# pengsongyou/openscene

Hardware: AMD Instinct MI355X
Metric: active voxels/sec MinkUNet18A fwd+bwd @2cm ScanNet; per-point query ms (higher is better)
Workload: dtype f32 (bf16x6 split-precision MFMA, fp32 accumulate); 1 GPU; ScanNet distillation step (configs[2]): MinkUNet18A, 768-d head, 1 synthetic S100k scene/GPU (100999 voxels on rank 0, 2 cm), training-mode BN; timed = coordinate+kernel maps, forward, cosine loss, backward, gradient all-reduce, Adam step; arch=MinkUNet18A, feature_dim=768, voxels_rank0=100999, parallelism=dp1

## Files before the change

### openscene_amd/csrc/bn.hip

```cpp
#include "common.h"
#include "epilogue.h"

namespace osn {

constexpr int CR_COLS = 64;
constexpr int CR_RL = 16;
constexpr int CR_MAX_BLOCKS = 512;

constexpr int BN_MAX_SRC = 3;
struct GySrc {
    const float* p[BN_MAX_SRC];
    int64_t ld[BN_MAX_SRC];
    int n;
};

__device__ inline float4 gy_load(const GySrc& s, int64_t r, int col) {
    float4 g = *reinterpret_cast<const float4*>(s.p[0] + r * s.ld[0] + col);
#pragma unroll
    for (int i = 1; i < BN_MAX_SRC; ++i)
        if (i < s.n) {
            const float4 v = *reinterpret_cast<const float4*>(s.p[i] + r * s.ld[i] + col);
            g.x += v.x; g.y += v.y; g.z += v.z; g.w += v.w;
        }
    return g;
}


struct ColReducePlan {
    int n_rb;
    int n_cg;
    int rows_per_block;
};

static ColReducePlan plan_colreduce(int64_t n, int c) {
    ColReducePlan p;
    p.n_cg = int(cdiv(c, CR_COLS));
    int64_t rb = cdiv(n, 4 * CR_RL);
    if (rb > CR_MAX_BLOCKS) rb = CR_MAX_BLOCKS;
    if (rb < 1) rb = 1;
    p.rows_per_block = int(cdiv(cdiv(n, rb), CR_RL) * CR_RL);
    p.n_rb = int(cdiv(n, p.rows_per_block));
    if (p.n_rb < 1) p.n_rb = 1;
    return p;
}

template <int MODE>
__global__ __launch_bounds__(256) void col_reduce_kernel(const float* __restrict__ x, const float* __restrict__ y,
                                                         const GySrc gy, const float* __restrict__ mean,
                                                         const float* __restrict__ var, float eps, int relu, int64_t n,
                                                         int c, int rows_per_block, double* __restrict__ partial,
                                                         const float* __restrict__ gamma, const float* __restrict__ beta) {
    __shared__ double red[2][CR_RL][CR_COLS];
    const int tid = threadIdx.x;
    const int cl = tid & 15, rl = tid >> 4;
    const int col = blockIdx.y * CR_COLS + cl * 4;
    const bool on = col < c;
    const int64_t r0 = int64_t(blockIdx.x) * rows_per_block;
    const int64_t r1 = min(n, r0 + rows_per_block);
    double s1[4] = {0, 0, 0, 0}, s2[4] = {0, 0, 0, 0};
    float4 mu = make_float4(0, 0, 0, 0), is = make_float4(0, 0, 0, 0);
    float4 ga = make_float4(0, 0, 0, 0), be = make_float4(0, 0, 0, 0);
    const bool from_x = MODE == 1 && relu && !y;
    if (MODE == 1 && on) {
        mu = *reinterpret_cast<const float4*>(mean + col);
        const float4 v = *reinterpret_cast<const float4*>(var + col);
        is = make_float4(bn_is(v.x, eps), bn_is(v.y, eps), bn_is(v.z, eps), bn_is(v.w, eps));
        if (from_x) {
            ga = *reinterpret_cast<const float4*>(gamma + col);
            be = *reinterpret_cast<const float4*>(beta + col);
        }
    }
    if (on) {
        for (int64_t r = r0 + rl; r < r1; r += CR_RL) {
            const float4 xv = *reinterpret_cast<const float4*>(x + r * c + col);
            if (MODE == 0) {
                s1[0] += xv.x; s1[1] += xv.y; s1[2] += xv.z; s1[3] += xv.w;
                s2[0] += double(xv.x) * xv.x; s2[1] += double(xv.y) * xv.y;
                s2[2] += double(xv.z) * xv.z; s2[3] += double(xv.w) * xv.w;
            } else {
                float4 g = gy_load(gy, r, col);
                if (from_x) {
                    g.x = bn_val(xv.x, mu.x, is.x, ga.x, be.x) > 0.f ? g.x : 0.f;
                    g.y = bn_val(xv.y, mu.y, is.y, ga.y, be.y) > 0.f ? g.y : 0.f;
                    g.z = bn_val(xv.z, mu.z, is.z, ga.z, be.z) > 0.f ? g.z : 0.f;
                    g.w = bn_val(xv.w, mu.w, is.w, ga.w, be.w) > 0.f ? g.w : 0.f;
                } else if (relu) {
                    const float4 yv = *reinterpret_cast<const float4*>(y + r * c + col);
                    g.x = yv.x > 0.f ? g.x : 0.f; g.y = yv.y > 0.f ? g.y : 0.f;
                    g.z = yv.z > 0.f ? g.z : 0.f; g.w = yv.w > 0.f ? g.w : 0.f;
                }
                s1[0] += g.x; s1[1] += g.y; s1[2] += g.z; s1[3] += g.w;
                s2[0] += double(g.x) * ((xv.x - mu.x) * is.x); s2[1] += double(g.y) * ((xv.y - mu.y) * is.y);
                s2[2] += double(g.z) * ((xv.z - mu.z) * is.z); s2[3] += double(g.w) * ((xv.w - mu.w) * is.w);
            }
        }
    }
#pragma unroll
    for (int j = 0; j < 4; ++j) {
        red[0][rl][cl * 4 + j] = s1[j];
        red[1][rl][cl * 4 + j] = s2[j];
    }
    __syncthreads();
    if (tid < 2 * CR_COLS) {
        const int which = tid / CR_COLS, cc = tid % CR_COLS;
        double s = 0;
#pragma unroll
        for (int r = 0; r < CR_RL; ++r) s += red[which][r][cc];
        const int gc = blockIdx.y * CR_COLS + cc;
        if (gc < c) partial[(int64_t(blockIdx.x) * 2 + which) * c + gc] = s;
    }
}

constexpr int FIN_COLS = 16, FIN_PARTS = 64;

constexpr int FIN_ITERS = CR_MAX_BLOCKS / FIN_PARTS;

__device__ inline void finalize_sums(const double* __restrict__ partial, int n_rb, int c, double& s1, double& s2,
                                     int& col) {
    __shared__ double red[2][FIN_PARTS][FIN_COLS];
    const int cl = threadIdx.x & (FIN_COLS - 1), part = threadIdx.x / FIN_COLS;
    col = blockIdx.x * FIN_COLS + cl;
    double va[FIN_ITERS], vb[FIN_ITERS];
    const int cc = col < c ? col : 0;
#pragma unroll
    for (int i = 0; i < FIN_ITERS; ++i) {
        const int blk = part + FIN_PARTS * i;
        const int bc = blk < n_rb ? blk : 0;
        va[i] = partial[(int64_t(bc) * 2 + 0) * c + cc];
        vb[i] = partial[(int64_t(bc) * 2 + 1) * c + cc];
    }
    double a = 0, b = 0;
#pragma unroll
    for (int i = 0; i < FIN_ITERS; ++i) {
        const bool on = col < c && part + FIN_PARTS * i < n_rb;
        a += on ? va[i] : 0.0;
        b += on ? vb[i] : 0.0;
    }
    red[0][part][cl] = a;
    red[1][part][cl] = b;
    __syncthreads();
    double t1 = 0, t2 = 0;
    if (part < 8) {
#pragma unroll
        for (int q = 0; q < 8; ++q) { t1 += red[0][part * 8 + q][cl]; t2 += red[1][part * 8 + q][cl]; }
    }
    __syncthreads();
    if (part < 8) {
        red[0][part][cl] = t1;
        red[1][part][cl] = t2;
    }
    __syncthreads();
    s1 = 0; s2 = 0;
    if (part == 0) {
#pragma unroll
        for (int q = 0; q < 8; ++q) { s1 += red[0][q][cl]; s2 += red[1][q][cl]; }
    }
}

__global__ __launch_bounds__(FIN_COLS * FIN_PARTS) void bn_stats_finalize_kernel(
    const double* __restrict__ partial, int n_rb, int64_t n, int c, float* __restrict__ mean, float* __restrict__ var,
    float* __restrict__ running_mean, float* __restrict__ running_var, float momentum) {
    double s1, s2;
    int j;
    finalize_sums(partial, n_rb, c, s1, s2, j);
    if (threadIdx.x >= FIN_COLS || j >= c) return;
    const double m = s1 / double(n);
    double v = s2 / double(n) - m * m;
    if (v < 0) v = 0;
    mean[j] = float(m);
    var[j] = float(v);
    if (running_mean) running_mean[j] = (1.f - momentum) * running_mean[j] + momentum * float(m);
    if (running_var) {
        const double unb = n > 1 ? v * double(n) / double(n - 1) : v;
        running_var[j] = (1.f - momentum) * running_var[j] + momentum * float(unb);
    }
}

__global__ __launch_bounds__(FIN_COLS * FIN_PARTS) void bn_bwd_finalize_kernel(const double* __restrict__ partial,
                                                                              int n_rb, int c,
                                                                              float* __restrict__ sum_g,
                                                                              float* __restrict__ sum_gx) {
    double s1, s2;
    int j;
    finalize_sums(partial, n_rb, c, s1, s2, j);
    if (threadIdx.x >= FIN_COLS || j >= c) return;
    sum_g[j] = float(s1);
    sum_gx[j] = float(s2);
}

__device__ inline float4 ld4(const float* p) { return *reinterpret_cast<const float4*>(p); }


__global__ __launch_bounds__(256) void bn_apply_kernel(const float* __restrict__ x, const float* __restrict__ mean,
                                                       const float* __restrict__ var, const float* __restrict__ gamma,
                                                       const float* __restrict__ beta, float eps,
                                                       const float* __restrict__ residual, int relu,
                                                       float* __restrict__ y, float* __restrict__ y2, int64_t ld2,
                                                       int64_t total4, int c4) {
    for (int64_t e = int64_t(blockIdx.x) * blockDim.x + threadIdx.x; e < total4; e += int64_t(gridDim.x) * blockDim.x) {
        const int col = int(e % c4) * 4;
        const float4 xv = ld4(x + e * 4), mu = ld4(mean + col), vv = ld4(var + col), ga = ld4(gamma + col),
                     be = ld4(beta + col);
        float4 o;
        o.x = bn_val(xv.x, mu.x, bn_is(vv.x, eps), ga.x, be.x);
        o.y = bn_val(xv.y, mu.y, bn_is(vv.y, eps), ga.y, be.y);
        o.z = bn_val(xv.z, mu.z, bn_is(vv.z, eps), ga.z, be.z);
        o.w = bn_val(xv.w, mu.w, bn_is(vv.w, eps), ga.w, be.w);
        if (residual) {
            const float4 rv = ld4(residual + e * 4);
            o.x += rv.x; o.y += rv.y; o.z += rv.z; o.w += rv.w;
        }
        if (relu) {
            o.x = bn_relu(o.x); o.y = bn_relu(o.y); o.z = bn_relu(o.z); o.w = bn_relu(o.w);
        }
        *reinterpret_cast<float4*>(y + e * 4) = o;
        if (y2) *reinterpret_cast<float4*>(y2 + (e / c4) * ld2 + col) = o;
    }
}

__global__ __launch_bounds__(256) void bn_bwd_apply_kernel(const float* __restrict__ x, const float* __restrict__ y,
                                                           const GySrc gy, const float* __restrict__ mean,
                                                           const float* __restrict__ var, const float* __restrict__ gamma,
                                                           float eps, int relu, int training,
                                                           const float* __restrict__ sum_g,
                                                           const float* __restrict__ sum_gx, float inv_n,
                                                           float* __restrict__ gx, float* __restrict__ gres,
                                                           int64_t total4, int c4, const float* __restrict__ beta) {
    const bool from_x = relu && !y;
    for (int64_t e = int64_t(blockIdx.x) * blockDim.x + threadIdx.x; e < total4; e += int64_t(gridDim.x) * blockDim.x) {
        const int col = int(e % c4) * 4;
        float4 g = gy_load(gy, e / c4, col);
        const float4 vv = ld4(var + col), ga = ld4(gamma + col);
        const float4 is = make_float4(bn_is(vv.x, eps), bn_is(vv.y, eps), bn_is(vv.z, eps), bn_is(vv.w, eps));
        float4 xv = make_float4(0, 0, 0, 0), mu = make_float4(0, 0, 0, 0);
        if (training || from_x) { xv = ld4(x + e * 4); mu = ld4(mean + col); }
        if (from_x) {
            const float4 be = ld4(beta + col);
            g.x = bn_val(xv.x, mu.x, is.x, ga.x, be.x) > 0.f ? g.x : 0.f;
            g.y = bn_val(xv.y, mu.y, is.y, ga.y, be.y) > 0.f ? g.y : 0.f;
            g.z = bn_val(xv.z, mu.z, is.z, ga.z, be.z) > 0.f ? g.z : 0.f;
            g.w = bn_val(xv.w, mu.w, is.w, ga.w, be.w) > 0.f ? g.w : 0.f;
        } else if (relu) {
            const float4 yv = ld4(y + e * 4);
            g.x = yv.x > 0.f ? g.x : 0.f; g.y = yv.y > 0.f ? g.y : 0.f;
            g.z = yv.z > 0.f ? g.z : 0.f; g.w = yv.w > 0.f ? g.w : 0.f;
        }
        if (gres) *reinterpret_cast<float4*>(gres + e * 4) = g;
        float4 o;
        if (training) {
            const float4 sg = ld4(sum_g + col), sx = ld4(sum_gx + col);
            o.x = ga.x * is.x * (g.x - sg.x * inv_n - (xv.x - mu.x) * is.x * sx.x * inv_n);
            o.y = ga.y * is.y * (g.y - sg.y * inv_n - (xv.y - mu.y) * is.y * sx.y * inv_n);
            o.z = ga.z * is.z * (g.z - sg.z * inv_n - (xv.z - mu.z) * is.z * sx.z * inv_n);
            o.w = ga.w * is.w * (g.w - sg.w * inv_n - (xv.w - mu.w) * is.w * sx.w * inv_n);
        } else {
            o.x = ga.x * is.x * g.x; o.y = ga.y * is.y * g.y; o.z = ga.z * is.z * g.z; o.w = ga.w * is.w * g.w;
        }
        *reinterpret_cast<float4*>(gx + e * 4) = o;
    }
}

constexpr int SB_THREADS = 1024, SB_RL = 512, SB_PER = 8, SB_COLS = 8;
constexpr int SB_MAX_ROWS = SB_RL * SB_PER;

__device__ inline double sb_wave_sum(double v) {
#pragma unroll
    for (int off = 2; off < 64; off <<= 1) v += __shfl_xor(v, off, 64);
    return v;
}

__device__ inline void sb_block_sums(double (&s)[8], int tid, int cl) {
    __shared__ double red[SB_THREADS / 64][2][8];
    __shared__ double tot[2][8];
#pragma unroll
    for (int q = 0; q < 8; ++q) s[q] = sb_wave_sum(s[q]);
    const int lane = tid & 63, wave = tid >> 6;
    if ((lane >> 1) == 0) {
#pragma unroll
        for (int q = 0; q < 8; ++q) red[wave][cl][q] = s[q];
    }
    __syncthreads();
    if (tid < 16) {
        const int c2 = tid >> 3, q = tid & 7;
        double t = 0;
#pragma unroll
        for (int w = 0; w < SB_THREADS / 64; ++w) t += red[w][c2][q];
        tot[c2][q] = t;
    }
    __syncthreads();
#pragma unroll
    for (int q = 0; q < 8; ++q) s[q] = tot[cl][q];
}

__global__ __launch_bounds__(SB_THREADS) void bn_small_fwd_kernel(const float* __restrict__ x, int n, int c,
                                                                  const float* __restrict__ gamma, const float* __restrict__ beta,
                                                                  float eps, const float* __restrict__ residual, int relu,
                                                                  float momentum, float* __restrict__ mean_out,
                                                                  float* __restrict__ var_out, float* __restrict__ running_mean,
                                                                  float* __restrict__ running_var, float* __restrict__ y,
                                                                  float* __restrict__ y2, int64_t ld2) {
    const int tid = threadIdx.x, cl = tid & 1, rl = tid >> 1;
    const int col = blockIdx.x * SB_COLS + cl * 4;
    const bool con = col < c;
    const int cc = con ? col : 0;
    float4 v[SB_PER];
    double s[8] = {0, 0, 0, 0, 0, 0, 0, 0};
#pragma unroll
    for (int j = 0; j < SB_PER; ++j) {
        const int r = rl + SB_RL * j;
        const bool ok = con && r < n;
        v[j] = ld4(x + int64_t(ok ? r : 0) * c + cc);
        if (ok) {
            s[0] += v[j].x; s[1] += v[j].y; s[2] += v[j].z; s[3] += v[j].w;
            s[4] += double(v[j].x) * v[j].x; s[5] += double(v[j].y) * v[j].y;
            s[6] += double(v[j].z) * v[j].z; s[7] += double(v[j].w) * v[j].w;
        }
    }
    sb_block_sums(s, tid, cl);
    float mu[4], vr[4];
#pragma unroll
    for (int q = 0; q < 4; ++q) {
        const double m = s[q] / double(n);
        double var = s[4 + q] / double(n) - m * m;
        if (var < 0) var = 0;
        mu[q] = float(m);
        vr[q] = float(var);
        if (rl == 0 && con) {
            mean_out[col + q] = mu[q];
            var_out[col + q] = vr[q];
            if (running_mean) running_mean[col + q] = (1.f - momentum) * running_mean[col + q] + momentum * mu[q];
            if (running_var) {
                const double unb = n > 1 ? var * double(n) / double(n - 1) : var;
                running_var[col + q] = (1.f - momentum) * running_var[col + q] + momentum * float(unb);
            }
        }
    }
    if (!con) return;
    const float4 ga = ld4(gamma + col), be = ld4(beta + col);
    const float is0 = bn_is(vr[0], eps), is1 = bn_is(vr[1], eps), is2 = bn_is(vr[2], eps), is3 = bn_is(vr[3], eps);
#pragma unroll
    for (int j = 0; j < SB_PER; ++j) {
        const int r = rl + SB_RL * j;
        if (r >= n) continue;
        float4 o;
        o.x = bn_val(v[j].x, mu[0], is0, ga.x, be.x);
        o.y = bn_val(v[j].y, mu[1], is1, ga.y, be.y);
        o.z = bn_val(v[j].z, mu[2], is2, ga.z, be.z);
        o.w = bn_val(v[j].w, mu[3], is3, ga.w, be.w);
        if (residual) {
            const float4 rv = ld4(residual + int64_t(r) * c + col);
            o.x += rv.x; o.y += rv.y; o.z += rv.z; o.w += rv.w;
        }
        if (relu) {
            o.x = bn_relu(o.x); o.y = bn_relu(o.y); o.z = bn_relu(o.z); o.w = bn_relu(o.w);
        }
        *reinterpret_cast<float4*>(y + int64_t(r) * c + col) = o;
        if (y2) *reinterpret_cast<float4*>(y2 + int64_t(r) * ld2 + col) = o;
    }
}

static int ew_grid(int64_t total4) {
    int64_t g = cdiv(total4, 256);
    if (g > 2048) g = 2048;
    if (g < 1) g = 1;
    return int(g);
}

}

using namespace osn;

extern "C" size_t osn_bn_ws_bytes(int64_t n, int c) {
    (void)n;
    return size_t(CR_MAX_BLOCKS) * 2 * size_t(c) * 8 + 256;
}

extern "C" int osn_bn_stats(const float* x, int64_t n, int c, float* mean, float* var, float* running_mean,
                            float* running_var, float momentum, void* ws, size_t ws_bytes, osn_stream_t stream) {
    hipStream_t st = static_cast<hipStream_t>(stream);
    OSN_REQUIRE(n >= 1 && c >= 4 && (c & 3) == 0, OSN_E_ARG, "osn_bn_stats: need n >= 1 and c %% 4 == 0 (n=%lld c=%d)", (long long)n, c);
    OSN_REQUIRE(x && mean && var && aligned16(x), OSN_E_ARG, "osn_bn_stats: null or unaligned pointer");
    ColReducePlan p = plan_colreduce(n, c);
    const size_t need = size_t(p.n_rb) * 2 * size_t(c) * 8;
    OSN_REQUIRE(ws && ws_bytes >= need, OSN_E_WS, "osn_bn_stats: workspace %zu < %zu", ws_bytes, need);
    double* partial = static_cast<double*>(ws);
    hipLaunchKernelGGL((col_reduce_kernel<0>), dim3(p.n_rb, p.n_cg), dim3(256), 0, st, x, (const float*)nullptr,
                       GySrc{}, (const float*)nullptr, (const float*)nullptr, 0.f, 0, n, c,
                       p.rows_per_block, partial, (const float*)nullptr, (const float*)nullptr);
    hipLaunchKernelGGL(bn_stats_finalize_kernel, dim3(cdiv(c, FIN_COLS)), dim3(FIN_COLS * FIN_PARTS), 0, st, partial, p.n_rb, n, c, mean, var,
                       running_mean, running_var, momentum);
    OSN_LAUNCH_CHECK();
    return OSN_OK;
}

extern "C" int osn_bn_apply2(const float* x, const float* mean, const float* var, const float* gamma, const float* beta,
                             float eps, const float* residual, int relu, float* y, float* y2, int64_t ld2, int64_t n, int c,
                             osn_stream_t stream) {
    hipStream_t st = static_cast<hipStream_t>(stream);
    OSN_REQUIRE(n >= 0 && c >= 4 && (c & 3) == 0, OSN_E_ARG, "osn_bn_apply: need c %% 4 == 0 (c=%d)", c);
    if (n == 0) return OSN_OK;
    OSN_REQUIRE(x && mean && var && gamma && beta && y, OSN_E_ARG, "osn_bn_apply: null pointer");
    OSN_REQUIRE(aligned16(x) && aligned16(y) && aligned16(mean) && aligned16(var) && aligned16(gamma) && aligned16(beta) &&
                    (!residual || aligned16(residual)),
                OSN_E_ARG, "osn_bn_apply: pointers must be 16-byte aligned");
    OSN_REQUIRE(!y2 || (aligned16(y2) && ld2 >= c && (ld2 & 3) == 0), OSN_E_ARG,
                "osn_bn_apply2: the second destination needs a 16-byte aligned pointer and a row stride >= c, %% 4 == 0");
    const int64_t total4 = n * (c / 4);
    hipLaunchKernelGGL(bn_apply_kernel, dim3(ew_grid(total4)), dim3(256), 0, st, x, mean, var, gamma, beta, eps,
                       residual, relu, y, y2, ld2, total4, c / 4);
    OSN_LAUNCH_CHECK();
    return OSN_OK;
}

extern "C" int osn_bn_apply(const float* x, const float* mean, const float* var, const float* gamma, const float* beta,
                            float eps, const float* residual, int relu, float* y, int64_t n, int c,
                            osn_stream_t stream) {
    return osn_bn_apply2(x, mean, var, gamma, beta, eps, residual, relu, y, nullptr, 0, n, c, stream);
}

extern "C" int osn_bn_forward_train2(const float* x, int64_t n, int c, const float* gamma, const float* beta, float eps,
                                     const float* residual, int relu, float momentum, float* mean, float* var,
                                     float* running_mean, float* running_var, float* y, float* y2, int64_t ld2, void* ws,
                                     size_t ws_bytes, osn_stream_t stream) {
    if (n >= 1 && n <= SB_MAX_ROWS && c >= 4 && (c & 3) == 0) {
        hipStream_t st = static_cast<hipStream_t>(stream);
        OSN_REQUIRE(x && mean && var && gamma && beta && y, OSN_E_ARG, "osn_bn_forward_train: null pointer");
        OSN_REQUIRE(aligned16(x) && aligned16(y) && aligned16(gamma) && aligned16(beta) && (!residual || aligned16(residual)),
                    OSN_E_ARG, "osn_bn_forward_train: pointers must be 16-byte aligned");
        OSN_REQUIRE(!y2 || (aligned16(y2) && ld2 >= c && (ld2 & 3) == 0), OSN_E_ARG,
                    "osn_bn_forward_train2: the second destination needs a 16-byte aligned pointer and a row stride >= c, %% 4 == 0");
        hipLaunchKernelGGL(bn_small_fwd_kernel, dim3(unsigned(cdiv(c, SB_COLS))), dim3(SB_THREADS), 0, st, x, int(n), c, gamma,
                           beta, eps, residual, relu, momentum, mean, var, running_mean, running_var, y, y2, ld2);
        OSN_LAUNCH_CHECK();
        return OSN_OK;
    }
    int rc = osn_bn_stats(x, n, c, mean, var, running_mean, running_var, momentum, ws, ws_bytes, stream);
    if (rc) return rc;
    return osn_bn_apply2(x, mean, var, gamma, beta, eps, residual, relu, y, y2, ld2, n, c, stream);
}

extern "C" int osn_bn_forward_train(const float* x, int64_t n, int c, const float* gamma, const float* beta, float eps,
                                    const float* residual, int relu, float momentum, float* mean, float* var,
                                    float* running_mean, float* running_var, float* y, void* ws, size_t ws_bytes,
                                    osn_stream_t stream) {
    return osn_bn_forward_train2(x, n, c, gamma, beta, eps, residual, relu, momentum, mean, var, running_mean, running_var, y,
                                 nullptr, 0, ws, ws_bytes, stream);
}

extern "C" int osn_bn_backward_multi2(const float* x, const float* y, const float* const* gy, const int64_t* gy_ld, int n_gy,
                                      const float* mean, const float* var, const float* gamma, const float* beta, float eps, int relu,
                                     int training, float* gx, float* gres, float* ggamma, float* gbeta, int64_t n, int c,
                                     void* ws, size_t ws_bytes, osn_stream_t stream) {
    hipStream_t st = static_cast<hipStream_t>(stream);
    OSN_REQUIRE(n >= 1 && c >= 4 && (c & 3) == 0, OSN_E_ARG, "osn_bn_backward: need n >= 1 and c %% 4 == 0");
    OSN_REQUIRE(gy && gy_ld && n_gy >= 1 && n_gy <= BN_MAX_SRC, OSN_E_ARG,
                "osn_bn_backward: %d gradient sources (1 .. %d are supported)", n_gy, BN_MAX_SRC);
    OSN_REQUIRE(x && mean && var && gamma && gx && ggamma && gbeta && (!relu || y || beta), OSN_E_ARG,
                "osn_bn_backward: null pointer");
    OSN_REQUIRE(!(relu && !y) || !gres, OSN_E_ARG, "osn_bn_backward: the ReLU mask can be recomputed from x only without a residual");
    OSN_REQUIRE(!beta || aligned16(beta), OSN_E_ARG, "osn_bn_backward: beta must be 16-byte aligned");
    OSN_REQUIRE(aligned16(x) && aligned16(gx) && aligned16(mean) && aligned16(var) && aligned16(gamma) &&
                    aligned16(ggamma) && aligned16(gbeta) && (!y || aligned16(y)) && (!gres || aligned16(gres)),
                OSN_E_ARG, "osn_bn_backward: pointers must be 16-byte aligned");
    GySrc src{};
    src.n = n_gy;
    for (int i = 0; i < BN_MAX_SRC; ++i) {
        const int j = i < n_gy ? i : 0;
        OSN_REQUIRE(gy[j] && aligned16(gy[j]) && gy_ld[j] >= c && (gy_ld[j] & 3) == 0, OSN_E_ARG,
                    "osn_bn_backward: gradient source %d needs a 16-byte aligned pointer and a row stride >= c, %% 4 == 0", j);
        src.p[i] = gy[j];
        src.ld[i] = gy_ld[j];
    }
    ColReducePlan p = plan_colreduce(n, c);
    const size_t need = size_t(p.n_rb) * 2 * size_t(c) * 8;
    OSN_REQUIRE(ws && ws_bytes >= need, OSN_E_WS, "osn_bn_backward: workspace %zu < %zu", ws_bytes, need);
    double* partial = static_cast<double*>(ws);
    hipLaunchKernelGGL((col_reduce_kernel<1>), dim3(p.n_rb, p.n_cg), dim3(256), 0, st, x, y, src, mean, var, eps, relu, n,
                       c, p.rows_per_block, partial, gamma, beta);
    hipLaunchKernelGGL(bn_bwd_finalize_kernel, dim3(cdiv(c, FIN_COLS)), dim3(FIN_COLS * FIN_PARTS), 0, st, partial, p.n_rb, c, gbeta, ggamma);
    const int64_t total4 = n * (c / 4);
    hipLaunchKernelGGL(bn_bwd_apply_kernel, dim3(ew_grid(total4)), dim3(256), 0, st, x, y, src, mean, var, gamma, eps,
                       relu, training, gbeta, ggamma, 1.f / float(n), gx, gres, total4, c / 4, beta);
    OSN_LAUNCH_CHECK();
    return OSN_OK;
}

extern "C" int osn_bn_backward_multi(const float* x, const float* y, const float* const* gy, const int64_t* gy_ld, int n_gy,
                                     const float* mean, const float* var, const float* gamma, float eps, int relu,
                                     int training, float* gx, float* gres, float* ggamma, float* gbeta, int64_t n, int c,
                                     void* ws, size_t ws_bytes, osn_stream_t stream) {
    OSN_REQUIRE(!relu || y, OSN_E_ARG, "osn_bn_backward_multi: relu needs y (or osn_bn_backward_multi2 with beta)");
    return osn_bn_backward_multi2(x, y, gy, gy_ld, n_gy, mean, var, gamma, nullptr, eps, relu, training, gx, gres, ggamma, gbeta, n, c,
                                  ws, ws_bytes, stream);
}

extern "C" int osn_bn_backward(const float* x, const float* y, const float* gy, const float* mean, const float* var,
                               const float* gamma, float eps, int relu, int training, float* gx, float* gres,
                               float* ggamma, float* gbeta, int64_t n, int c, void* ws, size_t ws_bytes,
                               osn_stream_t stream) {
    const int64_t ld = c;
    return osn_bn_backward_multi(x, y, &gy, &ld, 1, mean, var, gamma, eps, relu, training, gx, gres, ggamma, gbeta, n, c, ws,
                                 ws_bytes, stream);
}
```

### openscene_amd/csrc/net.hip

```cpp
#include "common.h"
#include <stdlib.h>
#include "events.h"
#include "epilogue.h"
#include <vector>

namespace osn {

constexpr uint64_t NO_OFF = ~uint64_t(0);

struct Events {
    std::vector<hipEvent_t> ev;
};

int events_count(const osn_events_t* e) { return e ? int(reinterpret_cast<const Events*>(e)->ev.size()) : 0; }
hipEvent_t events_get(const osn_events_t* e, int i) { return reinterpret_cast<const Events*>(e)->ev[size_t(i)]; }

struct Prof {
    std::vector<hipEvent_t> ev;
    std::vector<int32_t> tag;
    std::vector<int32_t> only;
    int cap = 0, n = 0;
};

static inline uint64_t up256(uint64_t x) { return (x + 255) & ~uint64_t(255); }
// ... 390 lines not shown
            OSN_HIP(hipEventRecord(evs->ev[net->n_ops + 1 + i], side));
            pending[i] = 1;
        }
    }
    for (int i = run->first_op; i < run->end_op; ++i)
        if (pending[i]) OSN_HIP(hipStreamWaitEvent(st, evs->ev[net->n_ops + 1 + i], 0));
    return OSN_OK;
}

extern "C" int osn_net_backward(const osn_net_desc* net, const osn_net_run* run, osn_stream_t stream) {
    OSN_REQUIRE(net && run, OSN_E_ARG, "osn_net_backward: null argument");
    Layout L;
    int rc = make_layout(net, run->level_rows, 1, L);
    if (rc) return rc;
    rc = check_run(net, run, L, true);
    if (rc) return rc;
    hipStream_t st = static_cast<hipStream_t>(stream);
    char* A = static_cast<char*>(run->fwd_arena);
    char* B = static_cast<char*>(run->bwd_arena);
    const int64_t* rows = run->level_rows;
    std::vector<osn_wgrad_job> jobs;
    jobs.reserve(size_t(net->n_ops));
    Events* evs = reinterpret_cast<Events*>(run->events);
    hipStream_t side = static_cast<hipStream_t>(run->side_stream);
    const bool forked = side && side != st && evs && int(evs->ev.size()) >= 2 * net->n_ops + 2 && run->ws_side &&
                        run->ws_side_bytes >= L.ws_bytes;
    osn_stream_t wstream = forked ? run->side_stream : stream;
    void* wws = forked ? run->ws_side : run->ws;
    const size_t wws_bytes = size_t(forked ? run->ws_side_bytes : run->ws_bytes);
    for (int i = run->end_op - 1; i >= run->first_op; --i) {
        const osn_net_op& o = net->ops[i];
        const int64_t n_in = rows[o.lvl_in], n_out = rows[o.lvl_out];
        const osn_net_weight& w = run->weights[o.weight];
        const float* gsrc[4];
        int64_t gld[4];
        int ng = 0;
        if (o.dst < 0) {
            OSN_REQUIRE(run->goutput || (run->goutput_rows && run->grows_pos && run->grows_idx && run->n_grows > 0), OSN_E_ARG,
                        "osn_net_backward: null output gradient");
            gsrc[ng] = run->goutput; gld[ng] = o.cout; ++ng;
        } else {
            for (int j = i + 1; j < net->n_ops && ng < 4; ++j) {
                const osn_net_op& c = net->ops[j];
                if (c.src == o.dst && c.need_dgrad) { gsrc[ng] = reinterpret_cast<const float*>(B + L.gin_off[j]); gld[ng] = c.cin; ++ng; }
                if (ng < 4 && c.res == o.dst) { gsrc[ng] = reinterpret_cast<const float*>(B + L.gres_off[j]); gld[ng] = c.cout; ++ng; }
                if (ng < 4 && o.copy_buf >= 0 && c.src == o.copy_buf && c.need_dgrad) {
                    gsrc[ng] = reinterpret_cast<const float*>(B + L.gin_off[j]) + o.copy_col; gld[ng] = c.cin; ++ng;
                }
            }
            OSN_REQUIRE(ng >= 1 && ng <= 3, OSN_E_ARG, "osn_net_backward: the output of op %d has %s consumers inside the executed range (1 .. 3 supported)",
                        i, ng == 0 ? "no" : "more than three");
        }
        const osn_net_run* r = run;
        const osn_stream_t sstream = stream;
        const float* gx;
        if (o.bn >= 0) {
            const osn_net_bn& bn = run->bns[o.bn];
            const float* x = reinterpret_cast<const float*>(A + L.x_off[i]);
            const float* y = reinterpret_cast<const float*>(A + L.y_off[o.dst]);
            const float *mean = bn.running_mean, *var = bn.running_var;
            if (run->training) {
                const float* mv = reinterpret_cast<const float*>(A + L.stat_off[i]);
                mean = mv; var = mv + o.cout;
            }
            float* gxw = reinterpret_cast<float*>(B + L.gx_off[i]);
            float* gres = o.res >= 0 ? reinterpret_cast<float*>(B + L.gres_off[i]) : nullptr;
            OSN_REQUIRE(bn.ggamma && bn.gbeta, OSN_E_ARG, "osn_net_backward: op %d: null batch-norm gradient pointers", i);
            const bool from_x = o.relu && o.res < 0 && bn.beta;
            rc = osn_bn_backward_multi2(x, from_x ? nullptr : y, gsrc, gld, ng, mean, var, bn.gamma, from_x ? bn.beta : nullptr, bn.eps,
                                        o.relu, run->training, gxw, gres, bn.ggamma, bn.gbeta, n_out, o.cout, r->ws, size_t(r->ws_bytes),
                                        sstream);
            if (rc) return rc;
            gx = gxw;
        } else {
            OSN_REQUIRE(ng == 1 && gld[0] == o.cout, OSN_E_ARG, "osn_net_backward: op %d without a batch norm needs one contiguous gradient", i);
            gx = gsrc[0];
        }
        const float* in = o.src < 0 ? run->input : reinterpret_cast<const float*>(A + L.y_off[o.src]);
        MapView v{};
        const osn_net_map* m = o.map >= 0 ? &run->maps[o.map] : nullptr;
        if (m) v = view_of(*m, o.transposed != 0);
        const bool sparse_rows = o.dst < 0 && o.K == 1 && o.bn < 0 && run->goutput_rows && run->grows_pos && run->grows_idx &&
                                 run->n_grows > 0 && run->n_grows < n_out && L.rows_in_off != NO_OFF &&
                                 (L.wgrad_k[i] == OSN_NET_K_WGRAD || L.wgrad_k[i] == OSN_NET_K_WGRAD_TL) &&
                                 (!o.need_dgrad || L.dgrad_k[i] == OSN_NET_K_DENSE);
        OSN_REQUIRE(o.dst >= 0 || sparse_rows || run->goutput, OSN_E_ARG,
                    "osn_net_backward: op %d: only the supervised rows of the output gradient were given, but the row-compacted head "
                    "backward does not apply to this configuration", i);
        OSN_REQUIRE(w.gW, OSN_E_ARG, "osn_net_backward: op %d: null weight-gradient pointer", i);
        if (forked && L.wgrad_k[i] == OSN_NET_K_WGRAD_STEM && !jobs.empty()) {
            rc = osn_wgrad_tl_reduce_batch(jobs.data(), int(jobs.size()), wstream);
            jobs.clear();
            if (rc) return rc;
        }
        const bool wg_main = forked && L.wgrad_k[i] == OSN_NET_K_WGRAD_STEM;
        if (forked && !wg_main) {
            OSN_HIP(hipEventRecord(evs->ev[i], st));
            OSN_HIP(hipStreamWaitEvent(side, evs->ev[i], 0));
        }
        {
            Bracket br(run->prof, i, 2, (forked && !wg_main) ? side : st);
            if (sparse_rows) {
                float* in_rows = reinterpret_cast<float*>(B + L.rows_in_off);
                rc = osn_rows_gather(in, run->grows_idx, run->n_grows, o.cin, in_rows, wstream);
                if (!rc)
                    rc = osn_spconv_wgrad(in_rows, run->goutput_rows, nullptr, nullptr, nullptr, w.gW, run->n_grows, 1, o.cin, o.cout, wws,
                                          wws_bytes, wstream);
            } else if (L.wgrad_k[i] == OSN_NET_K_WGRAD_TL) {
                OSN_REQUIRE(o.K == 1 || (m && m->pl_fwd), OSN_E_ARG, "osn_net_backward: op %d: pair lists missing", i);
                osn_wgrad_job job;
                rc = osn_spconv_wgrad_tl_partial(in, gx, m ? m->pl_fwd : nullptr, o.transposed ? 1 : 0, w.gW, n_in, n_out, o.K, o.cin, o.cout,
                                                 B + L.gpart_off[i], osn_spconv_wgrad_tl_ws_bytes(o.K, o.cin, o.cout), &job, wstream);
                if (!rc) jobs.push_back(job);
                if (!rc && forked && jobs.size() >= 12) {
                    rc = osn_wgrad_tl_reduce_batch(jobs.data(), int(jobs.size()), wstream);
                    jobs.clear();
                }
            } else if (L.wgrad_k[i] == OSN_NET_K_WGRAD_STEM) {
                OSN_REQUIRE(v.nbr_f, OSN_E_ARG, "osn_net_backward: op %d: the stem weight gradient needs the plain table", i);
                rc = wg_main ? osn_stem_conv_wgrad(in, gx, v.nbr_f, w.gW, n_out, o.K, o.cin, o.cout, run->ws, size_t(run->ws_bytes), stream)
                             : osn_stem_conv_wgrad(in, gx, v.nbr_f, w.gW, n_out, o.K, o.cin, o.cout, wws, wws_bytes, wstream);
            } else {
                rc = osn_spconv_wgrad(in, gx, o.K > 1 ? v.nbr_f : nullptr, o.K > 1 && m ? m->counts : nullptr, nullptr, w.gW, n_out, o.K,
                                      o.cin, o.cout, wws, wws_bytes, wstream);
            }
        }
        if (rc) return rc;
        if (o.need_dgrad) {
            float* gin = reinterpret_cast<float*>(B + L.gin_off[i]);
            {
                Bracket br(run->prof, i, 1, st);
                const int swap_f = o.transposed ? 1 : 0;
                if (sparse_rows) {
                    float* gin_rows = reinterpret_cast<float*>(B + L.rows_gin_off);
                    rc = osn_dense_fwd(run->goutput_rows, w.tl_dgrad, gin_rows, run->n_grows, o.cout, o.cin, sstream);
                    if (!rc) rc = osn_rows_scatter_zero(gin_rows, run->grows_pos, n_in, o.cin, gin, sstream);
                } else
                rc = run_conv(L.dgrad_k[i], gx, n_out, gin, n_in, o.K, o.cout, o.cin, nullptr, w.x6_dgrad, w.tl_dgrad, v.nbr_b, v.tb_rows,
                              v.tb_tbl, v.tb_g, v.tl_b, v.tl_b_rows, v.tl_b_bm, m ? m->pl_fwd : nullptr, o.transposed ? n_in : n_out,
                              (m && m->flip) ? swap_f : 1 - swap_f, r, sstream, i);
            }
            if (rc) return rc;
        }
    }
    rc = osn_wgrad_tl_reduce_batch(jobs.data(), int(jobs.size()), wstream);
    if (rc) return rc;
    if (forked && !(run->flags & OSN_NET_RUN_NO_JOIN)) {
        OSN_HIP(hipEventRecord(evs->ev[net->n_ops], side));
        OSN_HIP(hipStreamWaitEvent(st, evs->ev[net->n_ops], 0));
    }
    return OSN_OK;
}

extern "C" osn_events_t* osn_events_create(int n) {
    if (n < 1) return nullptr;
    Events* e = new (std::nothrow) Events();
    if (!e) return nullptr;
    e->ev.resize(size_t(n), nullptr);
    for (int i = 0; i < n; ++i) {
        if (hipEventCreateWithFlags(&e->ev[i], hipEventDisableTiming) != hipSuccess) {
            for (int j = 0; j < i; ++j) (void)hipEventDestroy(e->ev[j]);
            delete e;
            return nullptr;
        }
    }
    return reinterpret_cast<osn_events_t*>(e);
}

extern "C" void osn_events_destroy(osn_events_t* h) {
    Events* e = reinterpret_cast<Events*>(h);
    if (!e) return;
    for (hipEvent_t x : e->ev) (void)hipEventDestroy(x);
    delete e;
}

extern "C" osn_prof_t* osn_prof_create(int capacity) {
    if (capacity < 1) return nullptr;
    Prof* p = new (std::nothrow) Prof();
    if (!p) return nullptr;
    p->ev.resize(size_t(2) * capacity, nullptr);
    p->tag.assign(capacity, 0);
    for (int i = 0; i < 2 * capacity; ++i) {
        if (hipEventCreate(&p->ev[i]) != hipSuccess) {
            for (int j = 0; j < i; ++j) (void)hipEventDestroy(p->ev[j]);
            delete p;
            return nullptr;
        }
    }
    p->cap = capacity;
    return reinterpret_cast<osn_prof_t*>(p);
}

extern "C" void osn_prof_destroy(osn_prof_t* h) {
    Prof* p = reinterpret_cast<Prof*>(h);
    if (!p) return;
    for (hipEvent_t e : p->ev) (void)hipEventDestroy(e);
    delete p;
}

extern "C" int osn_prof_filter(osn_prof_t* h, const int32_t* tags, int n_tags) {
    Prof* p = reinterpret_cast<Prof*>(h);
    OSN_REQUIRE(p && n_tags >= 0 && (n_tags == 0 || tags), OSN_E_ARG, "osn_prof_filter: bad arguments");
    p->only.assign(tags, tags + n_tags);
    return OSN_OK;
}

extern "C" int osn_prof_read(osn_prof_t* h, int32_t* tags, float* ms, int capacity, int reset) {
    Prof* p = reinterpret_cast<Prof*>(h);
    if (!p || !tags || !ms) return 0;
    int n = p->n < capacity ? p->n : capacity;
    for (int i = 0; i < n; ++i) {
        float t = 0.f;
        if (hipEventSynchronize(p->ev[2 * i + 1]) != hipSuccess || hipEventElapsedTime(&t, p->ev[2 * i], p->ev[2 * i + 1]) != hipSuccess)
            t = -1.f;
        tags[i] = p->tag[i];
        ms[i] = t;
    }
    if (reset) p->n = 0;
    return n;
}
```

### openscene_amd/ops.py

```python
import ctypes
import os
import threading
import weakref

import torch

from . import _lib
from ._lib import check

_vp = ctypes.c_void_p

_profiler = None


def set_profiler(p):
    global _profiler
    _profiler = p


_raw_stream_of = torch._C._cuda_getCurrentRawStream
_current_device = torch._C._cuda_getDevice


def _prof_start(kind, dev, **meta):
# ... 769 lines not shown
    return bool(_cached("osn_spconv_fwd_x6_ok", int(n_out), int(K), int(cin), int(cout)))


def weight_transpose(weight, flip):
    dev = weight.device
    lib = _prep(dev)
    w = _f32c(_w3(weight), "weight")
    K, cin, cout = w.shape
    wt = torch.empty((K, cout, cin), dtype=torch.float32, device=dev)
    with _Dev(dev):
        check(lib.osn_weight_transpose(_p(w), K, cin, cout, int(bool(flip)), _p(wt), _stream(dev)),
              "osn_weight_transpose")
    return wt


_wgrad_items = {}


def _wgrad_plan_items(lib, counts, n_out, K, cin, cout, dev):
    nbytes = _cached("osn_spconv_wgrad_items_bytes", n_out, K, cin, cout)
    key = id(counts)
    hit = _wgrad_items.get(key)
    if hit is None or hit[0]() is not counts:
        hit = _wgrad_items[key] = (weakref.ref(counts, lambda _r, k=key: _wgrad_items.pop(k, None)), {})
    per_map = hit[1]
    sub = (int(n_out), int(K), int(cin), int(cout))
    items = per_map.get(sub)
    if items is None:
        items = per_map[sub] = torch.empty(nbytes // 4, dtype=torch.int32, device=dev)
        with _Dev(dev):
            check(lib.osn_spconv_wgrad_plan(_p(counts), n_out, K, cin, cout, _p(items), _stream(dev)),
                  "osn_spconv_wgrad_plan")
    return items


def spconv_wgrad(feats, gout, nbr, K, counts=None):
    dev = feats.device
    lib = _prep(dev)
    feats = _f32c(feats, "features")
    gout = _f32c(gout, "grad_output")
    n_out, cout = gout.shape
    cin = feats.shape[1]
    if nbr is not None:
        nbr = nbr.contiguous()
        if nbr.shape != (K, n_out):
            raise ValueError("nbr shape %s does not match (K=%d, n_out=%d)" % (tuple(nbr.shape), K, n_out))
    gw = torch.empty((K, cin, cout), dtype=torch.float32, device=dev)
    wsb = _cached("osn_spconv_wgrad_ws_bytes", n_out, K, cin, cout)
    ws = _ws(wsb, dev) if wsb else None
    tok = _prof_start("spconv_wgrad", dev, n_in=feats.shape[0], n_out=n_out, K=K, cin=cin, cout=cout)
    items = _wgrad_plan_items(lib, counts, n_out, K, cin, cout, dev) if (counts is not None and n_out > 0) else None
    with _Dev(dev):
        check(lib.osn_spconv_wgrad(_p(feats), _p(gout), _p(nbr), _p(counts), _p(items), _p(gw), n_out, K, cin, cout,
                                   _p(ws), int(wsb), _stream(dev)), "osn_spconv_wgrad")
    if tok is not None:
        _profiler.stop(tok)
    return gw


_plan_cache = {}


def spconv_fwd_plan(n_out, K, cin, cout):
    key = (int(n_out), int(K), int(cin), int(cout))
    v = _plan_cache.get(key)
    if v is None:
        plan = (ctypes.c_int32 * 6)()
        check(_lib.load().osn_spconv_fwd_plan(key[0], key[1], key[2], key[3], plan), "osn_spconv_fwd_plan")
        v = _plan_cache[key] = tuple(plan)
    return v


def bn_stats(x, running_mean=None, running_var=None, momentum=0.1):
    dev = x.device
    lib = _prep(dev)
    x = _f32c(x, "x")
    n, c = x.shape
    mean = torch.empty(c, dtype=torch.float32, device=dev)
    var = torch.empty(c, dtype=torch.float32, device=dev)
    wsb = _cached("osn_bn_ws_bytes", n, c)
    ws = _ws(wsb, dev)
    with _Dev(dev):
        check(lib.osn_bn_stats(_p(x), n, c, _p(mean), _p(var), _p(running_mean), _p(running_var), float(momentum),
                               _p(ws), ws.numel(), _stream(dev)), "osn_bn_stats")
    return mean, var


def bn_apply(x, mean, var, gamma, beta, eps, residual=None, relu=False):
    dev = x.device
    lib = _prep(dev)
    x = _f32c(x, "x")
    n, c = x.shape
    if residual is not None:
        residual = _f32c(residual, "residual")
        if residual.shape != x.shape:
            raise ValueError("residual shape %s != %s" % (tuple(residual.shape), tuple(x.shape)))
    y = torch.empty_like(x)
    with _Dev(dev):
        check(lib.osn_bn_apply(_p(x), _p(mean), _p(var), _p(gamma), _p(beta), float(eps), _p(residual), int(bool(relu)),
                               _p(y), n, c, _stream(dev)), "osn_bn_apply")
    return y


def bn_forward_train(x, gamma, beta, eps, residual, relu, running_mean, running_var, momentum):
    dev = x.device
    lib = _prep(dev)
    x = _f32c(x, "x")
    n, c = x.shape
    if residual is not None:
        residual = _f32c(residual, "residual")
        if residual.shape != x.shape:
            raise ValueError("residual shape %s != %s" % (tuple(residual.shape), tuple(x.shape)))
    mv = torch.empty((2, c), dtype=torch.float32, device=dev)
    y = torch.empty_like(x)
    ws = _ws(_cached("osn_bn_ws_bytes", n, c), dev)
    with _Dev(dev):
        check(lib.osn_bn_forward_train(_p(x), n, c, _p(gamma), _p(beta), float(eps), _p(residual), int(bool(relu)),
                                       float(momentum), _p(mv[0]), _p(mv[1]), _p(running_mean), _p(running_var), _p(y),
                                       _p(ws), ws.numel(), _stream(dev)), "osn_bn_forward_train")
    return y, mv[0], mv[1]


def bn_backward(x, y, gy, mean, var, gamma, eps, relu, training, want_gres, beta=None):
    return bn_backward_multi(x, y, [_f32c(gy, "grad_output")], mean, var, gamma, eps, relu, training, want_gres, beta=beta)


def _row_view(t, c, name):
    if t.dtype != torch.float32 or t.dim() != 2 or t.shape[1] != c or (t.shape[0] > 1 and t.stride(1) != 1):
        raise TypeError("%s must be a float32 [n, %d] matrix with unit column stride" % (name, c))
    ld = t.stride(0) if t.shape[0] > 1 else max(c, t.stride(0))
    if ld % 4 or t.data_ptr() % 16:
        raise ValueError("%s: row stride and first element must be 16-byte aligned" % name)
    return t.data_ptr(), ld


def bn_forward_train2(x, gamma, beta, eps, residual, relu, running_mean, running_var, momentum, y2):
    dev = x.device
    lib = _prep(dev)
    x = _f32c(x, "x")
    n, c = x.shape
    if residual is not None:
        residual = _f32c(residual, "residual")
    p2, ld2 = _row_view(y2, c, "y2")
    mv = torch.empty((2, c), dtype=torch.float32, device=dev)
    y = torch.empty_like(x)
    ws = _ws(_cached("osn_bn_ws_bytes", n, c), dev)
    with _Dev(dev):
        check(lib.osn_bn_forward_train2(_p(x), n, c, _p(gamma), _p(beta), float(eps), _p(residual), int(bool(relu)),
                                        float(momentum), _p(mv[0]), _p(mv[1]), _p(running_mean), _p(running_var), _p(y), p2, ld2,
                                        _p(ws), ws.numel(), _stream(dev)), "osn_bn_forward_train2")
    return y, mv[0], mv[1]


def bn_backward_multi(x, y, gys, mean, var, gamma, eps, relu, training, want_gres, beta=None):
    dev = x.device
    lib = _prep(dev)
    n, c = x.shape
    if relu and y is None and (beta is None or want_gres):
        raise ValueError("batch-norm backward with ReLU needs y, or beta and no residual")
    views = [_row_view(g, c, "grad_output[%d]" % i) for i, g in enumerate(gys)]
    ptrs = (ctypes.c_void_p * len(views))(*[v[0] for v in views])
    lds = (ctypes.c_int64 * len(views))(*[v[1] for v in views])
    gx = torch.empty_like(x)
    gres = torch.empty_like(x) if want_gres else None
    ggamma = torch.empty(c, dtype=torch.float32, device=dev)
    gbeta = torch.empty(c, dtype=torch.float32, device=dev)
    ws = _ws(_cached("osn_bn_ws_bytes", n, c), dev)
    with _Dev(dev):
        check(lib.osn_bn_backward_multi2(_p(x), _p(y), ptrs, lds, len(views), _p(mean), _p(var), _p(gamma),
                                         _p(beta) if (relu and y is None) else None, float(eps),
                                         int(bool(relu)), int(bool(training)), _p(gx), _p(gres), _p(ggamma), _p(gbeta), n, c,
                                         _p(ws), ws.numel(), _stream(dev)), "osn_bn_backward_multi2")
    return gx, gres, ggamma, gbeta


def relu_fwd(x):
    dev = x.device
    lib = _prep(dev)
    x = _f32c(x, "x")
    y = torch.empty_like(x)
    with _Dev(dev):
        check(lib.osn_relu_fwd(_p(x), _p(y), x.numel(), _stream(dev)), "osn_relu_fwd")
    return y


def relu_bwd(y, gy):
    dev = y.device
    lib = _prep(dev)
    gy = _f32c(gy, "grad_output")
    gx = torch.empty_like(y)
    with _Dev(dev):
        check(lib.osn_relu_bwd(_p(y), _p(gy), _p(gx), y.numel(), _stream(dev)), "osn_relu_bwd")
    return gx


def add(a, b):
    dev = a.device
    lib = _prep(dev)
    a, b = _f32c(a, "a"), _f32c(b, "b")
    if a.shape != b.shape:
        raise ValueError("add: shapes %s and %s differ" % (tuple(a.shape), tuple(b.shape)))
    out = torch.empty_like(a)
    with _Dev(dev):
        check(lib.osn_add(_p(a), _p(b), _p(out), a.numel(), _stream(dev)), "osn_add")
    return out


def cat2(a, b):
    dev = a.device
    lib = _prep(dev)
    a, b = _f32c(a, "a"), _f32c(b, "b")
    if a.dim() != 2 or b.dim() != 2 or a.shape[0] != b.shape[0]:
        raise ValueError("cat2: need two [n, c] matrices with equal n")
    n, ca, cb = a.shape[0], a.shape[1], b.shape[1]
    out = torch.empty((n, ca + cb), dtype=torch.float32, device=dev)
    with _Dev(dev):
        check(lib.osn_cat2(_p(a), ca, _p(b), cb, _p(out), n, _stream(dev)), "osn_cat2")
    return out


def cat2_bwd(gout, ca, cb):
    dev = gout.device
    lib = _prep(dev)
    gout = _f32c(gout, "grad_output")
    n = gout.shape[0]
    ga = torch.empty((n, ca), dtype=torch.float32, device=dev)
    gb = torch.empty((n, cb), dtype=torch.float32, device=dev)
    with _Dev(dev):
        check(lib.osn_cat2_bwd(_p(gout), _p(ga), ca, _p(gb), cb, n, _stream(dev)), "osn_cat2_bwd")
    return ga, gb


def cosine_query(feats, text_half, gather=None, want_scores=True):
    dev = feats.device
    lib = _prep(dev)
    feats = _query_feats(feats, "features")
    if text_half.dtype != torch.float16:
        raise TypeError("text features must be float16 (util/util.py:41-44 produces fp16)")
    text_half = text_half.contiguous()
    c, d = text_half.shape
    if feats.shape[1] != d:
        raise ValueError("feature dim %d != text dim %d" % (feats.shape[1], d))
    if gather is not None:
        if gather.dtype != torch.int64:
            gather = gather.long()
        gather = gather.contiguous()
        n = gather.shape[0]
    else:
        n = feats.shape[0]
    scores = torch.empty((n, c), dtype=torch.float16, device=dev) if want_scores else None
    amax = torch.empty(n, dtype=torch.int64, device=dev)
    with _Dev(dev):
        check(lib.osn_cosine_query(_p(feats), _p(gather), _p(text_half), _p(scores), _p(amax), n, d, c, _stream(dev)),
              "osn_cosine_query")
    return scores, amax


def query_ensemble(feat_distill, feat_fusion, text_half, gather_distill=None, gather_fusion=None, want_scores=True):
    dev = feat_distill.device
    lib = _prep(dev)
    fd = _query_feats(feat_distill, "distill features")
    ff = _query_feats(feat_fusion, "fusion features")
    text_half = text_half.contiguous()
    c, d = text_half.shape

    def _g(g):
        if g is None:
            return None
        return (g if g.dtype == torch.int64 else g.long()).contiguous()

    gd, gf = _g(gather_distill), _g(gather_fusion)
    n = gd.shape[0] if gd is not None else fd.shape[0]
    nf = gf.shape[0] if gf is not None else ff.shape[0]
    if n != nf:
        raise ValueError("the two feature sources address %d vs %d points" % (n, nf))
    scores = torch.empty((n, c), dtype=torch.float16, device=dev) if want_scores else None
    amax = torch.empty(n, dtype=torch.int64, device=dev)
    sel = torch.empty(n, dtype=torch.uint8, device=dev)
    wsb = lib.osn_query_ensemble_ws_bytes(n)
    ws = _ws(wsb, dev)
    with _Dev(dev):
        check(lib.osn_query_ensemble(_p(fd), _p(gd), _p(ff), _p(gf), _p(text_half), _p(scores), _p(amax), _p(sel), n,
                                     d, c, _p(ws), ws.numel(), _stream(dev)), "osn_query_ensemble")
    return scores, amax, sel.bool()


def _vote_matrix(votes, n, c, dev):
    if (votes.dtype != torch.float16 or votes.dim() != 2 or tuple(votes.shape) != (n, c) or votes.device != dev
            or not votes.is_contiguous()):
        raise ValueError("votes must be a contiguous float16 [%d, %d] matrix on the features' device" % (n, c))
    if votes.data_ptr() % (16 if c % 8 == 0 else 2):
        raise ValueError("votes must start 16-byte aligned when the label count is a multiple of 8")


def cosine_query_vote(feats, text_half, votes, gather=None, want_labels=False):
    dev = feats.device
    lib = _prep(dev)
    feats = _query_feats(feats, "features")
    if text_half.dtype != torch.float16:
        raise TypeError("text features must be float16 (util/util.py:41-44 produces fp16)")
    text_half = text_half.contiguous()
    c, d = text_half.shape
    if feats.shape[1] != d:
        raise ValueError("feature dim %d != text dim %d" % (feats.shape[1], d))
    if gather is not None:
        gather = (gather if gather.dtype == torch.int64 else gather.long()).contiguous()
    n = gather.shape[0] if gather is not None else feats.shape[0]
    _vote_matrix(votes, n, c, dev)
    amax = torch.empty(n, dtype=torch.int64, device=dev) if want_labels else None
    with _Dev(dev):
        check(lib.osn_cosine_query_vote(_p(feats), _p(gather), _p(text_half), _p(votes), _p(amax), n, d, c, _stream(dev)),
              "osn_cosine_query_vote")
    return amax


def query_ensemble_vote(feat_distill, feat_fusion, text_half, votes, gather_distill=None, gather_fusion=None, want_labels=False):
    dev = feat_distill.device
# ... 1015 lines not shown
```

Before: 12.37 million voxels/s.

## Store masked grad in BN backward reduce pass and reuse it in apply

When a residual gradient buffer is requested and does not alias the inputs, the backward column-reduce kernel now writes the combined, ReLU-masked gradient directly into gres. The apply kernel then reads that single buffer instead of re-summing up to three gradient sources and re-reading y or recomputing the ReLU mask. This trades a write during the reduce pass for fewer reads in the apply pass. Fork events also drop the system fence flag to make cross-stream sync cheaper, and the Python wrapper gains an optional preallocated gres output.

```diff
diff --git a/openscene_amd/csrc/bn.hip b/openscene_amd/csrc/bn.hip
--- a/openscene_amd/csrc/bn.hip
+++ b/openscene_amd/csrc/bn.hip
@@ -44,12 +44,13 @@
     return p;
 }
 
-template <int MODE>
-__global__ __launch_bounds__(256) void col_reduce_kernel(const float* __restrict__ x, const float* __restrict__ y,
-                                                         const GySrc gy, const float* __restrict__ mean,
-                                                         const float* __restrict__ var, float eps, int relu, int64_t n,
-                                                         int c, int rows_per_block, double* __restrict__ partial,
-                                                         const float* __restrict__ gamma, const float* __restrict__ beta) {
+template <int MODE, bool STORE_G>
+__device__ __forceinline__ void col_reduce_body(const float* __restrict__ x, const float* __restrict__ y, const GySrc gy,
+                                                const float* __restrict__ mean, const float* __restrict__ var, float eps,
+                                                int relu, int64_t n, int c, int rows_per_block, double* __restrict__ partial,
+                                                const float* __restrict__ gamma, const float* __restrict__ beta,
+                                                float* __restrict__ gres) {
+    static_assert(!STORE_G || MODE == 1, "only the backward sums form g");
     __shared__ double red[2][CR_RL][CR_COLS];
     const int tid = threadIdx.x;
     const int cl = tid & 15, rl = tid >> 4;
@@ -60,7 +61,7 @@
     double s1[4] = {0, 0, 0, 0}, s2[4] = {0, 0, 0, 0};
     float4 mu = make_float4(0, 0, 0, 0), is = make_float4(0, 0, 0, 0);
     float4 ga = make_float4(0, 0, 0, 0), be = make_float4(0, 0, 0, 0);
-    const bool from_x = MODE == 1 && relu && !y;
+    const bool from_x = MODE == 1 && !STORE_G && relu && !y;
     if (MODE == 1 && on) {
         mu = *reinterpret_cast<const float4*>(mean + col);
         const float4 v = *reinterpret_cast<const float4*>(var + col);
@@ -89,6 +90,7 @@
                     g.x = yv.x > 0.f ? g.x : 0.f; g.y = yv.y > 0.f ? g.y : 0.f;
                     g.z = yv.z > 0.f ? g.z : 0.f; g.w = yv.w > 0.f ? g.w : 0.f;
                 }
+                if (STORE_G) *reinterpret_cast<float4*>(gres + r * c + col) = g;
                 s1[0] += g.x; s1[1] += g.y; s1[2] += g.z; s1[3] += g.w;
                 s2[0] += double(g.x) * ((xv.x - mu.x) * is.x); s2[1] += double(g.y) * ((xv.y - mu.y) * is.y);
                 s2[2] += double(g.z) * ((xv.z - mu.z) * is.z); s2[3] += double(g.w) * ((xv.w - mu.w) * is.w);
@@ -109,6 +111,23 @@
         const int gc = blockIdx.y * CR_COLS + cc;
         if (gc < c) partial[(int64_t(blockIdx.x) * 2 + which) * c + gc] = s;
     }
+}
+
+template <int MODE>
+__global__ __launch_bounds__(256) void col_reduce_kernel(const float* __restrict__ x, const float* __restrict__ y,
+                                                         const GySrc gy, const float* __restrict__ mean,
+                                                         const float* __restrict__ var, float eps, int relu, int64_t n,
+                                                         int c, int rows_per_block, double* __restrict__ partial,
+                                                         const float* __restrict__ gamma, const float* __restrict__ beta) {
+    col_reduce_body<MODE, false>(x, y, gy, mean, var, eps, relu, n, c, rows_per_block, partial, gamma, beta, nullptr);
+}
+
+__global__ __launch_bounds__(256) void col_reduce_gres_kernel(const float* __restrict__ x, const float* __restrict__ y,
+                                                              const GySrc gy, const float* __restrict__ mean,
+                                                              const float* __restrict__ var, float eps, int relu, int64_t n,
+                                                              int c, int rows_per_block, double* __restrict__ partial,
+                                                              float* __restrict__ gres) {
+    col_reduce_body<1, true>(x, y, gy, mean, var, eps, relu, n, c, rows_per_block, partial, nullptr, nullptr, gres);
 }
 
 constexpr int FIN_COLS = 16, FIN_PARTS = 64;
@@ -218,23 +237,23 @@
     }
 }
 
-__global__ __launch_bounds__(256) void bn_bwd_apply_kernel(const float* __restrict__ x, const float* __restrict__ y,
-                                                           const GySrc gy, const float* __restrict__ mean,
-                                                           const float* __restrict__ var, const float* __restrict__ gamma,
-                                                           float eps, int relu, int training,
-                                                           const float* __restrict__ sum_g,
-                                                           const float* __restrict__ sum_gx, float inv_n,
-                                                           float* __restrict__ gx, float* __restrict__ gres,
-                                                           int64_t total4, int c4, const float* __restrict__ beta) {
-    const bool from_x = relu && !y;
+template <bool LOAD_G>
+__device__ __forceinline__ void bn_bwd_apply_body(const float* __restrict__ x, const float* __restrict__ y, const GySrc& gy,
+                                                  const float* __restrict__ mean, const float* __restrict__ var,
+                                                  const float* __restrict__ gamma, float eps, int relu, int training,
+                                                  const float* __restrict__ sum_g, const float* __restrict__ sum_gx, float inv_n,
+                                                  float* __restrict__ gx, float* __restrict__ gres, int64_t total4, int c4,
+                                                  const float* __restrict__ beta) {
+    const bool from_x = !LOAD_G && relu && !y;
     for (int64_t e = int64_t(blockIdx.x) * blockDim.x + threadIdx.x; e < total4; e += int64_t(gridDim.x) * blockDim.x) {
         const int col = int(e % c4) * 4;
-        float4 g = gy_load(gy, e / c4, col);
+        float4 g = LOAD_G ? ld4(gres + e * 4) : gy_load(gy, e / c4, col);
         const float4 vv = ld4(var + col), ga = ld4(gamma + col);
         const float4 is = make_float4(bn_is(vv.x, eps), bn_is(vv.y, eps), bn_is(vv.z, eps), bn_is(vv.w, eps));
         float4 xv = make_float4(0, 0, 0, 0), mu = make_float4(0, 0, 0, 0);
         if (training || from_x) { xv = ld4(x + e * 4); mu = ld4(mean + col); }
-        if (from_x) {
+        if (LOAD_G) {
+        } else if (from_x) {
             const float4 be = ld4(beta + col);
             g.x = bn_val(xv.x, mu.x, is.x, ga.x, be.x) > 0.f ? g.x : 0.f;
             g.y = bn_val(xv.y, mu.y, is.y, ga.y, be.y) > 0.f ? g.y : 0.f;
@@ -245,7 +264,7 @@
             g.x = yv.x > 0.f ? g.x : 0.f; g.y = yv.y > 0.f ? g.y : 0.f;
             g.z = yv.z > 0.f ? g.z : 0.f; g.w = yv.w > 0.f ? g.w : 0.f;
         }
-        if (gres) *reinterpret_cast<float4*>(gres + e * 4) = g;
+        if (!LOAD_G && gres) *reinterpret_cast<float4*>(gres + e * 4) = g;
         float4 o;
         if (training) {
             const float4 sg = ld4(sum_g + col), sx = ld4(sum_gx + col);
@@ -258,6 +277,27 @@
         }
         *reinterpret_cast<float4*>(gx + e * 4) = o;
     }
+}
+
+__global__ __launch_bounds__(256) void bn_bwd_apply_kernel(const float* __restrict__ x, const float* __restrict__ y,
+                                                           const GySrc gy, const float* __restrict__ mean,
+                                                           const float* __restrict__ var, const float* __restrict__ gamma,
+                                                           float eps, int relu, int training,
+                                                           const float* __restrict__ sum_g,
+                                                           const float* __restrict__ sum_gx, float inv_n,
+                                                           float* __restrict__ gx, float* __restrict__ gres,
+                                                           int64_t total4, int c4, const float* __restrict__ beta) {
+    bn_bwd_apply_body<false>(x, y, gy, mean, var, gamma, eps, relu, training, sum_g, sum_gx, inv_n, gx, gres, total4, c4, beta);
+}
+
+__global__ __launch_bounds__(256) void bn_bwd_apply_gres_kernel(const float* __restrict__ x, const float* __restrict__ mean,
+                                                                const float* __restrict__ var, const float* __restrict__ gamma,
+                                                                float eps, int training, const float* __restrict__ sum_g,
+                                                                const float* __restrict__ sum_gx, float inv_n,
+                                                                float* __restrict__ gx, const float* __restrict__ gres,
+                                                                int64_t total4, int c4) {
+    bn_bwd_apply_body<true>(x, nullptr, GySrc{}, mean, var, gamma, eps, 0, training, sum_g, sum_gx, inv_n, gx,
+                            const_cast<float*>(gres), total4, c4, nullptr);
 }
 
 constexpr int SB_THREADS = 1024, SB_RL = 512, SB_PER = 8, SB_COLS = 8;
@@ -357,6 +397,11 @@
         *reinterpret_cast<float4*>(y + int64_t(r) * c + col) = o;
         if (y2) *reinterpret_cast<float4*>(y2 + int64_t(r) * ld2 + col) = o;
     }
+}
+
+static bool ranges_overlap(const float* a, size_t na, const float* b, size_t nb) {
+    const uintptr_t a0 = reinterpret_cast<uintptr_t>(a), b0 = reinterpret_cast<uintptr_t>(b);
+    return a0 < b0 + nb * sizeof(float) && b0 < a0 + na * sizeof(float);
 }
 
 static int ew_grid(int64_t total4) {
@@ -475,12 +520,26 @@
     const size_t need = size_t(p.n_rb) * 2 * size_t(c) * 8;
     OSN_REQUIRE(ws && ws_bytes >= need, OSN_E_WS, "osn_bn_backward: workspace %zu < %zu", ws_bytes, need);
     double* partial = static_cast<double*>(ws);
-    hipLaunchKernelGGL((col_reduce_kernel<1>), dim3(p.n_rb, p.n_cg), dim3(256), 0, st, x, y, src, mean, var, eps, relu, n,
-                       c, p.rows_per_block, partial, gamma, beta);
+    const size_t span = size_t(n) * size_t(c);
+    bool via_gres = gres != nullptr && !ranges_overlap(gres, span, x, span) && !(y && ranges_overlap(gres, span, y, span)) &&
+                    !ranges_overlap(gres, span, gx, span);
+    for (int i = 0; via_gres && i < n_gy; ++i)
+        via_gres = !ranges_overlap(gres, span, src.p[i], size_t(n - 1) * size_t(src.ld[i]) + size_t(c));
+    const dim3 rgrid(p.n_rb, p.n_cg);
+    if (via_gres)
+        hipLaunchKernelGGL(col_reduce_gres_kernel, rgrid, dim3(256), 0, st, x, y, src, mean, var, eps, relu, n, c,
+                           p.rows_per_block, partial, gres);
+    else
+        hipLaunchKernelGGL((col_reduce_kernel<1>), rgrid, dim3(256), 0, st, x, y, src, mean, var, eps, relu, n, c,
+                           p.rows_per_block, partial, gamma, beta);
     hipLaunchKernelGGL(bn_bwd_finalize_kernel, dim3(cdiv(c, FIN_COLS)), dim3(FIN_COLS * FIN_PARTS), 0, st, partial, p.n_rb, c, gbeta, ggamma);
     const int64_t total4 = n * (c / 4);
-    hipLaunchKernelGGL(bn_bwd_apply_kernel, dim3(ew_grid(total4)), dim3(256), 0, st, x, y, src, mean, var, gamma, eps,
-                       relu, training, gbeta, ggamma, 1.f / float(n), gx, gres, total4, c / 4, beta);
+    if (via_gres)
+        hipLaunchKernelGGL(bn_bwd_apply_gres_kernel, dim3(ew_grid(total4)), dim3(256), 0, st, x, mean, var, gamma, eps, training,
+                           gbeta, ggamma, 1.f / float(n), gx, (const float*)gres, total4, c / 4);
+    else
+        hipLaunchKernelGGL(bn_bwd_apply_kernel, dim3(ew_grid(total4)), dim3(256), 0, st, x, y, src, mean, var, gamma, eps,
+                           relu, training, gbeta, ggamma, 1.f / float(n), gx, gres, total4, c / 4, beta);
     OSN_LAUNCH_CHECK();
     return OSN_OK;
 }
diff --git a/openscene_amd/csrc/net.hip b/openscene_amd/csrc/net.hip
--- a/openscene_amd/csrc/net.hip
+++ b/openscene_amd/csrc/net.hip
@@ -566,13 +566,17 @@
     return OSN_OK;
 }
 
+#ifndef OSN_FORK_EVENT_FLAGS
+#define OSN_FORK_EVENT_FLAGS (hipEventDisableTiming | hipEventDisableSystemFence)
+#endif
+
 extern "C" osn_events_t* osn_events_create(int n) {
     if (n < 1) return nullptr;
     Events* e = new (std::nothrow) Events();
     if (!e) return nullptr;
     e->ev.resize(size_t(n), nullptr);
     for (int i = 0; i < n; ++i) {
-        if (hipEventCreateWithFlags(&e->ev[i], hipEventDisableTiming) != hipSuccess) {
+        if (hipEventCreateWithFlags(&e->ev[i], OSN_FORK_EVENT_FLAGS) != hipSuccess) {
             for (int j = 0; j < i; ++j) (void)hipEventDestroy(e->ev[j]);
             delete e;
             return nullptr;
diff --git a/openscene_amd/ops.py b/openscene_amd/ops.py
--- a/openscene_amd/ops.py
+++ b/openscene_amd/ops.py
@@ -945,7 +945,7 @@
     return y, mv[0], mv[1]
 
 
-def bn_backward_multi(x, y, gys, mean, var, gamma, eps, relu, training, want_gres, beta=None):
+def bn_backward_multi(x, y, gys, mean, var, gamma, eps, relu, training, want_gres, beta=None, gres_out=None):
     dev = x.device
     lib = _prep(dev)
     n, c = x.shape
@@ -955,7 +955,10 @@
     ptrs = (ctypes.c_void_p * len(views))(*[v[0] for v in views])
     lds = (ctypes.c_int64 * len(views))(*[v[1] for v in views])
     gx = torch.empty_like(x)
-    gres = torch.empty_like(x) if want_gres else None
+    if gres_out is not None and (not want_gres or gres_out.dtype != torch.float32 or gres_out.shape != x.shape or
+                                 gres_out.device != dev or not gres_out.is_contiguous()):
+        raise ValueError("gres_out must be a contiguous float32 tensor shaped like x, on its device, and needs want_gres")
+    gres = (gres_out if gres_out is not None else torch.empty_like(x)) if want_gres else None
     ggamma = torch.empty(c, dtype=torch.float32, device=dev)
     gbeta = torch.empty(c, dtype=torch.float32, device=dev)
     ws = _ws(_cached("osn_bn_ws_bytes", n, c), dev)
```

After: 12.62 million voxels/s (median of 6 runs). +2.1%, better.
